# PeterouZh/CIPS-3Dplusplus

Measured on AMD Instinct MI355X. Metric: rendered views/sec at FFHQ 1024^2 (generator forward: 64x64-ray NeRF + StyleGAN2 decoder), higher is better.
Workload: dtype f32 (split-fp16 MFMA products x3, f32 accumulate and storage); 1 GPU; ffhq_r1024_nerf64x64x24_D2_B1_fp32; img_size=64, n_samples=24, N_layers_renderer=2, resolution=1024, parallelism=views x1, views_in_flight=2

## Files before the change

### cips_3dplusplus_amd/csrc/chain.hip

```cpp
#include "mfma_frag.h"

namespace {

#ifdef CIPS3D_CHAIN_STAMPS
__device__ unsigned long long g_chain_stamps[8];
extern "C" int cips3d_debug_read_chain_stamps(unsigned long long* out8) {
  hipDeviceSynchronize();
  hipMemcpyFromSymbol(out8, HIP_SYMBOL(g_chain_stamps), 64);
  unsigned long long z[8] = {0};
  hipMemcpyToSymbol(HIP_SYMBOL(g_chain_stamps), z, 64);
  return 0;
}
#define CSTAMP(i) ts_[i] = __builtin_amdgcn_s_memtime()
#else
#define CSTAMP(i)
#endif

struct ChainArgs {
  const _Float16* x;
  const float* wmp;
  void* out;
  int out_fmt;
  int B, Cin, Cout; int HW;
  int epilogue; const float* noise; int64_t noise_bstride; const float* noise_w; const float* bias;
  const float* rgb_w; float* rgb_part;
  const int* x_exp; int x_exp_const; const float* x_pmax; float x_max_const; const float* lconst; float* out_amax; int* out_exp;
  float* out_pmax;
  cips3d_reduce_job ride;
};



template <int WM, int WGM, int WGN, int BK, int NS, int NP = 2>
__global__ void __launch_bounds__(64 * WGM * WGN) chain_gemm_kernel(ChainArgs a) {
#ifdef CIPS3D_CHAIN_STAMPS
  unsigned long long ts_[6];
  CSTAMP(0);
#endif
  constexpr int NW = WGM * WGN;
  constexpr int BM = 16 * WM * WGM, BN = 64 * WGN;
  constexpr int A_STAGE = BM * BK * NP / 2, B_STAGE = BK * BN * NP / 2, STAGE = A_STAGE + B_STAGE;
  constexpr int A_PIECES = A_STAGE / 256, B_PIECES = B_STAGE / 256, PIECES = A_PIECES + B_PIECES;
  constexpr int PW = PIECES / NW;
  constexpr int KB = BK / 32, KQ = KB * NP;
  static_assert(PIECES % NW == 0 && BK % 32 == 0, "tile shape");
  static_assert(NP != 2 || BN == CIPS3D_PLANES_EXP_BLOCK, "one planes exponent per workgroup pixel block");
  __shared__ __attribute__((aligned(16))) float lds[NS * STAGE];

  const int tid = threadIdx.x;
  const int wave = __builtin_amdgcn_readfirstlane(tid >> 6);
  const int lane = tid & 63;
  const int wm_i = wave / WGN, wn_i = wave % WGN;
  const int q = lane >> 4, col = lane & 15;
  const int b = blockIdx.z;

  if constexpr (NP == 2) {
    if (a.ride.part && (int)blockIdx.y == a.Cout / BM) {
      constexpr int RIDE_K = 12;
      const int64_t wv = ((int64_t)blockIdx.z * gridDim.x + blockIdx.x) * NW + wave;
      const int64_t ride_i = wv * 16 + col;
      const bool ride_on = ride_i < a.ride.n4;
      f32x4 rsl[RIDE_K], rsk = {0.f, 0.f, 0.f, 0.f};
#pragma unroll
      for (int k = 0; k < RIDE_K; ++k)
        rsl[k] = (ride_on && q + 4 * k < a.ride.n_slots)
                     ? *reinterpret_cast<const f32x4*>(a.ride.part + (q + 4 * k) * a.ride.slot_stride + ride_i * 4)
                     : f32x4{0.f, 0.f, 0.f, 0.f};
      if (ride_on && a.ride.skip && q == 0) rsk = *reinterpret_cast<const f32x4*>(a.ride.skip + ride_i * 4);
      f32x4 v = {0.f, 0.f, 0.f, 0.f};
#pragma unroll
      for (int it = 0; it < RIDE_K / 4; ++it)
        if (q + 16 * it < a.ride.n_slots) {
#pragma unroll
          for (int u = 0; u < 4; ++u)
#pragma unroll
            for (int c = 0; c < 4; ++c) v[c] += rsl[4 * it + u][c];
        }
#pragma unroll
      for (int g = 1; g < 4; ++g)
#pragma unroll
        for (int c = 0; c < 4; ++c) {
          const float o = __shfl(v[c], col + 16 * g, 64);
          if (q == 0) v[c] += o;
        }
      if (ride_on && q == 0) {
        const int ch = (int)((ride_i / a.ride.HW4) % 3);
        float bs = 0.f;
        for (int k = 0; k < a.ride.n_bias; ++k) bs += a.ride.bias[k][ch];
#pragma unroll
        for (int c = 0; c < 4; ++c) v[c] += bs;
        if (a.ride.skip) {
#pragma unroll
          for (int c = 0; c < 4; ++c) v[c] += rsk[c];
        }
        *reinterpret_cast<f32x4*>(a.ride.out + ride_i * 4) = v;
      }
      return;
    }
  }
  const int m0 = blockIdx.y * BM, n0 = blockIdx.x * BN;
  const int HW = a.HW, K = a.Cin;
  const int nstage = K / BK;
  float* s_part = lds + (nstage % NS) * STAGE;
  const _Float16* xb = a.x + (int64_t)b * K * HW * NP;
  const float* ab = a.wmp + (int64_t)b * a.Cout * K * NP / 2;

  auto stage_load = [&](int st) {
    float* dstA = lds + (st % NS) * STAGE;
    float* dstB = dstA + A_STAGE;
    const int k0 = st * BK;
#pragma unroll
    for (int j = 0; j < PW; ++j) {
      const int piece = j * NW + wave;
      if (piece < A_PIECES) {
        const int ot_l = piece / KQ, kq_l = piece % KQ;
        const char* ub = reinterpret_cast<const char*>(ab + ((((m0 >> 4) + ot_l) * ((K >> 5) * NP) + (k0 >> 5) * NP + kq_l) * 256));
        unsigned vo = lane * 16;
        asm volatile("" : "+s"(ub), "+v"(vo));
        __builtin_amdgcn_global_load_lds((const __attribute__((address_space(1))) void*)(ub + vo),
                                         (__attribute__((address_space(3))) void*)(dstA + piece * 256), 16, 0, 0);
      } else {
        const int pb = piece - A_PIECES;
        const int row = pb / (BN / 64), chunk = pb % (BN / 64);
        int n = n0 + chunk * 64 + lane;
        if (n > HW - 1) n = HW - 1;
        const char* ub = reinterpret_cast<const char*>(xb + ((int64_t)((k0 >> 3) * NP + row) * HW) * 8);
        unsigned vo = (unsigned)n * 16u;
        asm volatile("" : "+s"(ub), "+v"(vo));
        __builtin_amdgcn_global_load_lds((const __attribute__((address_space(1))) void*)(ub + vo),
                                         (__attribute__((address_space(3))) void*)(dstB + pb * 256), 16, 0, 0);
      }
    }
  };

  const int nl = wn_i * 64 + col;
  int npx[4];
#pragma unroll
  for (int c = 0; c < 4; ++c) npx[c] = n0 + nl + 16 * c;

  float nz[4] = {0.f, 0.f, 0.f, 0.f};
  f32x4 bias4[WM];
  f32x4 wrgb[WM][3];
  float nw = 0.f;
  float kin = NP == 2 ? kSplitInv : 1.f;
  float kout = 1.f, kback = 1.f;
  float lc0 = 0.f, lc1 = 0.f;
  float pin = 0.f;
  const bool track = NP == 2 && a.out_fmt == 1 && a.lconst;
  int e_raw = 0;
  f32x4 lc_raw = {0.f, 0.f, 0.f, 0.f};
  auto issue_ops = [&]() {
    if constexpr (NP == 2) {
      const int nblk = (HW + BN - 1) / BN;
      if (a.x_exp) {
        typedef const __attribute__((address_space(1))) int gi32_t;
        e_raw = __hip_atomic_load(reinterpret_cast<gi32_t*>(reinterpret_cast<uintptr_t>(a.x_exp + b * nblk + blockIdx.x)),
                                  __ATOMIC_RELAXED, __HIP_MEMORY_SCOPE_AGENT);
      }
      if (track) {
        const float* lc = a.lconst + b * 4;
        lc_raw = f32x4{lc[0], lc[1], lc[2], 0.f};
        if (a.x_pmax) {
          const int n_half = (HW + 63) / 64, per = K >> 4;
          const int n_ent = (2 * (int)blockIdx.x + 1 < n_half ? 2 : 1) * per;
          const float* pp = a.x_pmax + ((int64_t)b * n_half + 2 * blockIdx.x) * per;
          if (lane < n_ent) pin = pp[lane];
        }
      }
    }
    if (a.epilogue == 1) {
      if (a.noise && a.noise_w) {
        nw = a.noise_w[0];
        const float* nzp = a.noise + (int64_t)b * a.noise_bstride;
#pragma unroll
        for (int c = 0; c < 4; ++c)
          if (npx[c] < HW) nz[c] = nzp[npx[c]];
      }
#pragma unroll
      for (int i = 0; i < WM; ++i)
        bias4[i] = *reinterpret_cast<const f32x4*>(a.bias + m0 + (wm_i * WM + i) * 16 + 4 * q);
    }
    if (a.rgb_part) {
#pragma unroll
      for (int i = 0; i < WM; ++i)
#pragma unroll
        for (int ch = 0; ch < 3; ++ch)
          wrgb[i][ch] = *reinterpret_cast<const f32x4*>(a.rgb_w + (int64_t)b * 3 * a.Cout + ch * a.Cout + m0 + (wm_i * WM + i) * 16 + 4 * q);
    }
  };
  auto finish_ops = [&]() {
    if constexpr (NP == 2) {
      const int e_in = a.x_exp ? __builtin_amdgcn_readfirstlane(e_raw) : a.x_exp_const;
      kin = cips3d_uniform(kin * cips3d_pow2(e_in));
      if (track) {
        lc0 = lc_raw[0];
        lc1 = fmaxf(lc_raw[1], 1.41421356237309515f * lc_raw[2]);
        if (a.x_pmax) {
          const int n_half = (HW + 63) / 64, per = K >> 4;
          const int n_ent = (2 * (int)blockIdx.x + 1 < n_half ? 2 : 1) * per;
          const float* pp = a.x_pmax + ((int64_t)b * n_half + 2 * blockIdx.x) * per;
          for (int i = lane + 64; i < n_ent; i += 64) pin = fmaxf(pin, pp[i]);
        } else {
          pin = a.x_max_const > 0.f ? a.x_max_const : cips3d_pow2(e_in + 15);
        }
      }
    }
  };
  f32x4 acc[WM][4];
#pragma unroll
  for (int i = 0; i < WM; ++i)
#pragma unroll
    for (int c = 0; c < 4; ++c) acc[i][c] = f32x4{0.f, 0.f, 0.f, 0.f};

  static_assert(NS >= 2 && (NS - 2) * PW <= 63, "counted vmcnt");
  if (NS > 2) issue_ops();
#pragma unroll
  for (int s0 = 0; s0 < NS - 1; ++s0)
    if (s0 < nstage) stage_load(s0);
  if (NS == 2) issue_ops();

#ifdef CIPS3D_CHAIN_STAMPS
  unsigned long long ph_[4] = {0, 0, 0, 0}, tp_ = __builtin_amdgcn_s_memtime();
#define PSTAMP(i) do { const unsigned long long t_ = __builtin_amdgcn_s_memtime(); ph_[i] += t_ - tp_; tp_ = t_; } while (0)
#else
#define PSTAMP(i)
#endif
  for (int st = 0; st < nstage; ++st) {
    int younger = nstage - 1 - st;
    if (younger > NS - 2) younger = NS - 2;
    switch (younger) {
      case 0: __builtin_amdgcn_s_waitcnt(vmcnt_imm(0)); break;
      case 1: __builtin_amdgcn_s_waitcnt(vmcnt_imm(PW)); break;
      case 2: __builtin_amdgcn_s_waitcnt(vmcnt_imm(2 * PW)); break;
      case 3: __builtin_amdgcn_s_waitcnt(vmcnt_imm(3 * PW)); break;
      case 4: __builtin_amdgcn_s_waitcnt(vmcnt_imm(4 * PW)); break;
      default: __builtin_amdgcn_s_waitcnt(vmcnt_imm(5 * PW)); break;
    }
    __builtin_amdgcn_s_barrier();
#ifdef CIPS3D_CHAIN_STAMPS
    if (st == 0) CSTAMP(1);
#endif
    if (st + NS - 1 < nstage) stage_load(st + NS - 1);
    PSTAMP(1);
    const float* sA = lds + (st % NS) * STAGE;
    const float* sB = sA + A_STAGE;
    if constexpr (NP == 2) {
      h8 ah[KB][WM], al[KB][WM], bh[KB][4], bl[KB][4];
#pragma unroll
      for (int kb = 0; kb < KB; ++kb) {
#pragma unroll
        for (int i = 0; i < WM; ++i) {
          ah[kb][i] = *reinterpret_cast<const h8*>(sA + ((wm_i * WM + i) * KQ + 2 * kb) * 256 + lane * 4);
          al[kb][i] = *reinterpret_cast<const h8*>(sA + ((wm_i * WM + i) * KQ + 2 * kb + 1) * 256 + lane * 4);
        }
#pragma unroll
        for (int c = 0; c < 4; ++c) {
          bh[kb][c] = *reinterpret_cast<const h8*>(sB + (((kb * 4 + q) * 2 + 0) * BN + nl + 16 * c) * 4);
          bl[kb][c] = *reinterpret_cast<const h8*>(sB + (((kb * 4 + q) * 2 + 1) * BN + nl + 16 * c) * 4);
        }
      }
      __builtin_amdgcn_sched_barrier(0);
#pragma unroll
      for (int kb = 0; kb < KB; ++kb)
#pragma unroll
        for (int i = 0; i < WM; ++i)
#pragma unroll
          for (int c = 0; c < 4; ++c) {
            acc[i][c] = __builtin_amdgcn_mfma_f32_16x16x32_f16(al[kb][i], bh[kb][c], acc[i][c], 0, 0, 0);
            acc[i][c] = __builtin_amdgcn_mfma_f32_16x16x32_f16(ah[kb][i], bl[kb][c], acc[i][c], 0, 0, 0);
            acc[i][c] = __builtin_amdgcn_mfma_f32_16x16x32_f16(ah[kb][i], bh[kb][c], acc[i][c], 0, 0, 0);
          }
    } else {
      bf8 af[KB][WM], bf[KB][4];
#pragma unroll
      for (int kb = 0; kb < KB; ++kb) {
#pragma unroll
        for (int i = 0; i < WM; ++i)
          af[kb][i] = *reinterpret_cast<const bf8*>(sA + ((wm_i * WM + i) * KQ + kb) * 256 + lane * 4);
#pragma unroll
        for (int c = 0; c < 4; ++c)
          bf[kb][c] = *reinterpret_cast<const bf8*>(sB + ((kb * 4 + q) * BN + nl + 16 * c) * 4);
      }
      __builtin_amdgcn_sched_barrier(0);
#pragma unroll
      for (int kb = 0; kb < KB; ++kb)
#pragma unroll
        for (int i = 0; i < WM; ++i)
#pragma unroll
          for (int c = 0; c < 4; ++c)
            acc[i][c] = __builtin_amdgcn_mfma_f32_16x16x32_bf16(af[kb][i], bf[kb][c], acc[i][c], 0, 0, 0);
    }
    PSTAMP(2);
    asm volatile("s_waitcnt lgkmcnt(0)" ::: "memory");
  }

  CSTAMP(2);
  finish_ops();
  if (track) {
    const float m_in = cips3d_wave_max_uniform(pin);
    const int e = cips3d_split_exp(fmaf(lc1, m_in * 1.000001f, lc0));
    kout = cips3d_uniform(cips3d_pow2(-e));
    kback = cips3d_uniform(cips3d_pow2(e));
    if (blockIdx.y == 0 && tid == 0) a.out_exp[b * ((HW + BN - 1) / BN) + blockIdx.x] = e;
  }
  float prgb[WM][3][4];
#pragma unroll
  for (int i = 0; i < WM; ++i)
#pragma unroll
    for (int ch = 0; ch < 3; ++ch)
#pragma unroll
      for (int c = 0; c < 4; ++c) prgb[i][ch][c] = 0.f;
  const float kact = 1.41421356237309515f * kout;
  const float kpre = a.epilogue == 1 ? kin : kin * kout;
  float mx = 0.f;
#pragma unroll
  for (int i = 0; i < WM; ++i) {
    const int obase = m0 + (wm_i * WM + i) * 16;
#pragma unroll
    for (int c = 0; c < 4; ++c) {
      float v[4];
#pragma unroll
      for (int r = 0; r < 4; ++r) {
        v[r] = acc[i][c][r] * kpre;
        if (a.epilogue == 1) v[r] = lrelu02(fmaf(nw, nz[c], v[r]) + bias4[i][r]) * kact;
      }
      mx = fmaxf(fmaxf(fabsf(v[0]), fabsf(v[1])), fmaxf(fmaxf(fabsf(v[2]), fabsf(v[3])), mx));
      if (a.rgb_part) {
#pragma unroll
        for (int ch = 0; ch < 3; ++ch)
#pragma unroll
          for (int r = 0; r < 4; ++r)
            asm volatile("v_fmac_f32 %0, %1, %2" : "+v"(prgb[i][ch][c]) : "v"(wrgb[i][ch][r]), "v"(v[r]));
      }
      if (npx[c] < HW) {
        if (a.out_fmt == 1) {
          h4 hi, lo;
          split_frag(v[0], v[1], v[2], v[3], hi, lo);
          _Float16* dst = reinterpret_cast<_Float16*>(a.out) +
                          ((((int64_t)b * (a.Cout >> 3) + (obase >> 3) + (q >> 1)) * 2) * HW + npx[c]) * 8 + 4 * (q & 1);
          cips3d_store_wt8(dst, hi);
          cips3d_store_wt8(dst + (int64_t)HW * 8, lo);
        } else if (a.out_fmt == 3) {
          unsigned short* dst = reinterpret_cast<unsigned short*>(a.out) +
                                (((int64_t)b * (a.Cout >> 3) + (obase >> 3) + (q >> 1)) * HW + npx[c]) * 8 + 4 * (q & 1);
          cips3d_store_wt8(dst, pack_bf16(v[0], v[1], v[2], v[3]));
        } else if (a.out_fmt == 2) {
          unsigned short* dst = reinterpret_cast<unsigned short*>(a.out) + ((int64_t)b * a.Cout + obase + 4 * q) * HW + npx[c];
          typedef __bf16 bf16x2_t __attribute__((ext_vector_type(2)));
          typedef float f32x2_t __attribute__((ext_vector_type(2)));
#pragma unroll
          for (int r = 0; r < 4; r += 2) {
            const bf16x2_t p = __builtin_convertvector(f32x2_t{v[r], v[r + 1]}, bf16x2_t);
            const unsigned bits = __builtin_bit_cast(unsigned, p);
            dst[(int64_t)r * HW] = (unsigned short)(bits & 0xffffu);
            dst[(int64_t)(r + 1) * HW] = (unsigned short)(bits >> 16);
          }
        } else {
          float* dst = reinterpret_cast<float*>(a.out) + ((int64_t)b * a.Cout + obase + 4 * q) * HW + npx[c];
#pragma unroll
          for (int r = 0; r < 4; ++r) cips3d_store_wt(dst + (int64_t)r * HW, v[r]);
        }
      }
    }
  }
#ifdef CIPS3D_CHAIN_STAMPS
  CSTAMP(3);
  __builtin_amdgcn_s_waitcnt(vmcnt_imm(0));
  CSTAMP(4);
  if (tid == 0) {
    for (int i = 0; i < 4; ++i) atomicAdd(&g_chain_stamps[i], ts_[i + 1] - ts_[i]);
    atomicAdd(&g_chain_stamps[7], 1ull);
    atomicAdd(&g_chain_stamps[4], ph_[0]);
    atomicAdd(&g_chain_stamps[5], ph_[1]);
    atomicAdd(&g_chain_stamps[6], ph_[2]);
  }
#endif
  if (a.out_pmax && n0 + wn_i * 64 < HW) {
    static_assert(BN == 64 * WGN, "a wave column = one 64-pixel half block");
    const float m = cips3d_wave_max_uniform(mx * kback);
    if (lane < WM)
      a.out_pmax[((int64_t)b * ((HW + 63) / 64) + (n0 >> 6) + wn_i) * (a.Cout >> 4) + (m0 >> 4) + wm_i * WM + lane] = m;
  }
  if (a.out_amax) {
    const float m = cips3d_workgroup_max(mx * kback, s_part, wave, lane, NW);
    if (tid == 0) cips3d_amax_raise_if(a.out_amax + b * CIPS3D_AMAX_FLOATS, m, blockIdx.y * gridDim.x + blockIdx.x);
  }
  if (!a.rgb_part) return;
#pragma unroll
  for (int i = 0; i < WM; ++i)
#pragma unroll
    for (int ch = 0; ch < 3; ++ch)
#pragma unroll
      for (int c = 0; c < 4; ++c) {
        float v = prgb[i][ch][c] * kback;
        v += __shfl_xor(v, 16, 64);
        v += __shfl_xor(v, 32, 64);
        prgb[i][ch][c] = v;
      }
  __syncthreads();
  float* s_red = lds;
  if (q == 0) {
#pragma unroll
    for (int i = 0; i < WM; ++i)
#pragma unroll
      for (int ch = 0; ch < 3; ++ch)
#pragma unroll
        for (int c = 0; c < 4; ++c) s_red[((wm_i * WM + i) * 3 + ch) * BN + nl + 16 * c] = prgb[i][ch][c];
  }
  __syncthreads();
  constexpr int SLOTS = BM / 64;
  static_assert(WGM * WM == 4 * SLOTS, "four tiles per ToRGB slot");
  if (wm_i < SLOTS && q < 3) {
#pragma unroll
    for (int c = 0; c < 4; ++c) {
      if (npx[c] >= HW) continue;
      float v = 0.f;
#pragma unroll
      for (int m = 0; m < 4; ++m) v += s_red[((wm_i * 4 + m) * 3 + q) * BN + nl + 16 * c];
      cips3d_store_wt(a.rgb_part + (((int64_t)blockIdx.y * SLOTS + wm_i) * a.B + b) * 3 * HW + ((int64_t)q * HW + npx[c]), v);
    }
  }
}

__device__ __forceinline__ float amax_of_sample(const float* __restrict__ slots) {
  float m = 0.f;
  for (int s_ = 0; s_ < CIPS3D_AMAX_SLOTS; ++s_) m = fmaxf(m, slots[s_ * CIPS3D_AMAX_STRIDE]);
  return m;
}

__global__ void __launch_bounds__(256) to_planes_kernel(const float* __restrict__ x, _Float16* __restrict__ p, int B, int C,
                                                        int HW, const float* __restrict__ x_amax, int* __restrict__ exp_out,
                                                        float* __restrict__ pmax_out) {
  const int64_t total = (int64_t)B * (C / 8) * HW, per = (int64_t)(C / 8) * HW;
  for (int64_t i = (int64_t)blockIdx.x * blockDim.x + threadIdx.x; i < total; i += (int64_t)gridDim.x * blockDim.x) {
    const int n = (int)(i % HW);
    const int64_t bc = i / HW;
    float k = 1.f;
    if (x_amax) {
      const int b = (int)(i / per);
      const int e_ = cips3d_split_exp(amax_of_sample(x_amax + (int64_t)b * CIPS3D_AMAX_FLOATS));
      k = cips3d_pow2(-e_);
      const int nblk = (HW + CIPS3D_PLANES_EXP_BLOCK - 1) / CIPS3D_PLANES_EXP_BLOCK;
      if (i - b * per < nblk) exp_out[b * nblk + (int)(i - b * per)] = e_;
      if (pmax_out) {
        const int n_pm = ((HW + 63) / 64) * (C >> 4);
        const float am = amax_of_sample(x_amax + (int64_t)b * CIPS3D_AMAX_FLOATS);
        for (int64_t j = i - b * per; j < n_pm; j += per) pmax_out[(int64_t)b * n_pm + j] = am;
      }
    }
    h8 hi, lo;
#pragma unroll
    for (int e = 0; e < 8; ++e) {
      const float v = x[(bc * 8 + e) * HW + n] * k;
      _Float16 h_, l_;
      cips3d_split16(v, h_, l_);
      hi[e] = h_;
      lo[e] = l_;
    }
    *reinterpret_cast<h8*>(p + ((bc * 2) * HW + n) * 8) = hi;
    *reinterpret_cast<h8*>(p + ((bc * 2 + 1) * HW + n) * 8) = lo;
  }
}

__global__ void __launch_bounds__(256) from_planes_kernel(const _Float16* __restrict__ p, float* __restrict__ x, int B, int C,
                                                          int HW, const int* __restrict__ exps) {
  const int64_t total = (int64_t)B * (C / 8) * HW, per = (int64_t)(C / 8) * HW;
  for (int64_t i = (int64_t)blockIdx.x * blockDim.x + threadIdx.x; i < total; i += (int64_t)gridDim.x * blockDim.x) {
    const int n = (int)(i % HW);
    const int64_t bc = i / HW;
    const float k = exps ? cips3d_pow2(exps[(i / per) * ((HW + CIPS3D_PLANES_EXP_BLOCK - 1) / CIPS3D_PLANES_EXP_BLOCK) +
                                            n / CIPS3D_PLANES_EXP_BLOCK]) : 1.f;
    const h8 hi = *reinterpret_cast<const h8*>(p + ((bc * 2) * HW + n) * 8);
    const h8 lo = *reinterpret_cast<const h8*>(p + ((bc * 2 + 1) * HW + n) * 8);
#pragma unroll
    for (int e = 0; e < 8; ++e) x[(bc * 8 + e) * HW + n] = ((float)hi[e] + (float)lo[e]) * k;
  }
}

__global__ void __launch_bounds__(256) to_planes16_kernel(const float* __restrict__ x, unsigned short* __restrict__ p, int B,
                                                          int C, int HW) {
  typedef __bf16 bf16x2_t __attribute__((ext_vector_type(2)));
  typedef float f32x2_t __attribute__((ext_vector_type(2)));
  typedef unsigned u32x4_t __attribute__((ext_vector_type(4)));
  const int64_t total = (int64_t)B * (C / 8) * HW;
  for (int64_t i = (int64_t)blockIdx.x * blockDim.x + threadIdx.x; i < total; i += (int64_t)gridDim.x * blockDim.x) {
    const int n = (int)(i % HW);
    const int64_t bc = i / HW;
    u32x4_t w;
#pragma unroll
    for (int e = 0; e < 8; e += 2) {
      const bf16x2_t pr = __builtin_convertvector(f32x2_t{x[(bc * 8 + e) * HW + n], x[(bc * 8 + e + 1) * HW + n]}, bf16x2_t);
      w[e >> 1] = __builtin_bit_cast(unsigned, pr);
    }
    *reinterpret_cast<u32x4_t*>(p + (bc * HW + n) * 8) = w;
  }
}

__global__ void __launch_bounds__(256) from_planes16_kernel(const unsigned short* __restrict__ p, float* __restrict__ x, int B,
                                                            int C, int HW) {
  typedef unsigned u32x4_t __attribute__((ext_vector_type(4)));
  const int64_t total = (int64_t)B * (C / 8) * HW;
  for (int64_t i = (int64_t)blockIdx.x * blockDim.x + threadIdx.x; i < total; i += (int64_t)gridDim.x * blockDim.x) {
    const int n = (int)(i % HW);
    const int64_t bc = i / HW;
    const u32x4_t w = *reinterpret_cast<const u32x4_t*>(p + (bc * HW + n) * 8);
#pragma unroll
    for (int e = 0; e < 8; e += 2) {
      x[(bc * 8 + e) * HW + n] = __uint_as_float(w[e >> 1] << 16);
      x[(bc * 8 + e + 1) * HW + n] = __uint_as_float(w[e >> 1] & 0xffff0000u);
    }
  }
}

}

extern "C" int cips3d_planes_supported(int Cin, int Cout, int64_t HW) {
  return Cin > 0 && Cout > 0 && Cin % 64 == 0 && Cout % 64 == 0 && HW >= 16 &&
         (int64_t)(Cin > Cout ? Cin : Cout) * HW * 2 + 1024 < ((int64_t)1 << 31);
}

extern "C" int cips3d_planes_torgb_blocks(int Cout) { return Cout > 0 ? Cout / 64 : 0; }

extern "C" int cips3d_to_planes(const float* x, void* planes, int B, int C, int64_t HW, const float* x_amax, int32_t* exp_out,
                                float* pmax_out, void* stream) {
  if (!x || !planes || B < 0 || C <= 0 || HW <= 0 || ((x_amax == nullptr) != (exp_out == nullptr)) || (pmax_out && !x_amax))
    return CIPS3D_E_BADARG;
  if (pmax_out && C % 16 != 0) return CIPS3D_E_UNSUPP;
  if (C % 8 != 0) return CIPS3D_E_UNSUPP;
  if (B == 0) return 0;
  int64_t blocks = ceil_div<int64_t>((int64_t)B * (C / 8) * HW, 256);
  if (blocks > 16384) blocks = 16384;
  hipLaunchKernelGGL(to_planes_kernel, dim3((unsigned)blocks), dim3(256), 0, as_stream(stream), x,
                     reinterpret_cast<_Float16*>(planes), B, C, (int)HW, x_amax, exp_out, pmax_out);
  return cips3d_launch_status();
}

extern "C" int cips3d_from_planes(const void* planes, float* x, int B, int C, int64_t HW, const int32_t* exp, void* stream) {
  if (!x || !planes || B < 0 || C <= 0 || HW <= 0) return CIPS3D_E_BADARG;
  if (C % 8 != 0) return CIPS3D_E_UNSUPP;
  if (B == 0) return 0;
  int64_t blocks = ceil_div<int64_t>((int64_t)B * (C / 8) * HW, 256);
  if (blocks > 16384) blocks = 16384;
  hipLaunchKernelGGL(from_planes_kernel, dim3((unsigned)blocks), dim3(256), 0, as_stream(stream),
                     reinterpret_cast<const _Float16*>(planes), x, B, C, (int)HW, exp);
  return cips3d_launch_status();
}

extern "C" int cips3d_to_planes16(const float* x, void* planes16, int B, int C, int64_t HW, void* stream) {
  if (!x || !planes16 || B < 0 || C <= 0 || HW <= 0) return CIPS3D_E_BADARG;
  if (C % 8 != 0) return CIPS3D_E_UNSUPP;
  if (B == 0) return 0;
  int64_t blocks = ceil_div<int64_t>((int64_t)B * (C / 8) * HW, 256);
  if (blocks > 16384) blocks = 16384;
  hipLaunchKernelGGL(to_planes16_kernel, dim3((unsigned)blocks), dim3(256), 0, as_stream(stream), x,
                     reinterpret_cast<unsigned short*>(planes16), B, C, (int)HW);
  return cips3d_launch_status();
}

extern "C" int cips3d_from_planes16(const void* planes16, float* x, int B, int C, int64_t HW, void* stream) {
  if (!x || !planes16 || B < 0 || C <= 0 || HW <= 0) return CIPS3D_E_BADARG;
  if (C % 8 != 0) return CIPS3D_E_UNSUPP;
  if (B == 0) return 0;
  int64_t blocks = ceil_div<int64_t>((int64_t)B * (C / 8) * HW, 256);
  if (blocks > 16384) blocks = 16384;
  hipLaunchKernelGGL(from_planes16_kernel, dim3((unsigned)blocks), dim3(256), 0, as_stream(stream),
                     reinterpret_cast<const unsigned short*>(planes16), x, B, C, (int)HW);
  return cips3d_launch_status();
}

extern "C" int cips3d_modconv1x1_planes16(const void* x_planes16, const float* wm, void* out, int out_format, int B, int Cin,
                                          int Cout, int64_t HW, int epilogue, const float* noise, int64_t noise_bstride,
                                          const float* noise_w, const float* bias, const float* rgb_w, float* rgb_part,
                                          int* n_row_blocks, const cips3d_range* rg, void* stream) {
  if ((rgb_w == nullptr) != (rgb_part == nullptr)) return CIPS3D_E_BADARG;
  if (n_row_blocks) *n_row_blocks = cips3d_planes_torgb_blocks(Cout);
  if (!x_planes16 || !wm || !out || B < 0 || Cin <= 0 || Cout <= 0 || HW <= 0) return CIPS3D_E_BADARG;
  if ((out_format != 0 && out_format != 2 && out_format != 3) || (epilogue != 0 && epilogue != 1) || (epilogue == 1 && !bias))
    return CIPS3D_E_BADARG;
  if (!cips3d_planes_supported(Cin, Cout, HW)) return CIPS3D_E_UNSUPP;
  if (B == 0) return 0;
  ChainArgs a{reinterpret_cast<const _Float16*>(x_planes16), wm, out, out_format, B, Cin, Cout, (int)HW, epilogue, noise,
              noise_bstride, noise_w, bias, rgb_w, rgb_part, nullptr, 0, nullptr, 0.f, nullptr, rg ? rg->out_amax : nullptr, nullptr,
              nullptr, cips3d_reduce_job{}};
  if (rg && rg->ride) return CIPS3D_E_UNSUPP;
  dim3 grid((unsigned)ceil_div<int64_t>(HW, 128), (unsigned)(Cout / 64), (unsigned)B);
  hipLaunchKernelGGL((chain_gemm_kernel<1, 4, 2, 64, 3, 1>), grid, dim3(512), 0, as_stream(stream), a);
  return cips3d_launch_status();
}

extern "C" int cips3d_modconv1x1_planes(const void* x_planes, const float* wm, void* out, int out_format, int B, int Cin,
                                        int Cout, int64_t HW, int epilogue, const float* noise, int64_t noise_bstride,
                                        const float* noise_w, const float* bias, const float* rgb_w, float* rgb_part,
                                        int* n_row_blocks, const cips3d_range* rg, void* stream) {
  if ((rgb_w == nullptr) != (rgb_part == nullptr)) return CIPS3D_E_BADARG;
  if (n_row_blocks) *n_row_blocks = cips3d_planes_torgb_blocks(Cout);
  if (!x_planes || !wm || !out || B < 0 || Cin <= 0 || Cout <= 0 || HW <= 0) return CIPS3D_E_BADARG;
  if (out_format < 0 || out_format > 2 || (epilogue != 0 && epilogue != 1) || (epilogue == 1 && !bias)) return CIPS3D_E_BADARG;
  if (!cips3d_planes_supported(Cin, Cout, HW)) return CIPS3D_E_UNSUPP;
  if (B == 0) return 0;
  if (rg && out_format == 1 && (!rg->lconst || !rg->out_exp)) return CIPS3D_E_BADARG;
  ChainArgs a{reinterpret_cast<const _Float16*>(x_planes), wm, out, out_format, B, Cin, Cout, (int)HW, epilogue, noise,
              noise_bstride, noise_w, bias, rgb_w, rgb_part, rg ? rg->x_exp : nullptr, rg ? rg->x_exp_const : 0,
              rg ? rg->x_pmax : nullptr, rg ? rg->x_max_const : 0.f, (rg && out_format == 1) ? rg->lconst : nullptr,
              (rg && out_format != 1) ? rg->out_amax : nullptr, rg ? rg->out_exp : nullptr,
              (rg && out_format == 1) ? rg->out_pmax : nullptr, cips3d_reduce_job{}};
  if (rg && out_format == 1 && rg->x_pmax && Cin > 512) return CIPS3D_E_UNSUPP;
  if (rg && rg->ride) {
    const cips3d_reduce_job& j = *rg->ride;
    if (!j.part || !j.out || j.n_slots < 1 || j.n_bias < 0 || j.n_bias > CIPS3D_TORGB_FOLD_MAX || j.n4 <= 0 || j.HW4 <= 0 ||
        j.slot_stride <= 0)
      return CIPS3D_E_BADARG;
    if (j.n_slots > 48 || j.n4 > (int64_t)ceil_div<int64_t>(HW, 128) * B * 8 * 16) return CIPS3D_E_UNSUPP;
    a.ride = j;
  }
  const int64_t tiles64 = (int64_t)B * (Cout / 64) * ceil_div<int64_t>(HW, 128);
  if (rg && rg->half_chip && Cout % 128 == 0 && tiles64 > 192 && tiles64 <= 256) {
    dim3 grid2((unsigned)ceil_div<int64_t>(HW, 128), (unsigned)(Cout / 128) + (a.ride.part ? 1u : 0u), (unsigned)B);
    hipLaunchKernelGGL((chain_gemm_kernel<2, 4, 2, 64, 2>), grid2, dim3(512), 0, as_stream(stream), a);
    return cips3d_launch_status();
  }
  dim3 grid((unsigned)ceil_div<int64_t>(HW, 128), (unsigned)(Cout / 64) + (a.ride.part ? 1u : 0u), (unsigned)B);
  hipLaunchKernelGGL((chain_gemm_kernel<1, 4, 2, 64, 2>), grid, dim3(512), 0, as_stream(stream), a);
  return cips3d_launch_status();
}
```

Measured before the change: 3435 views/s.

## Software-pipeline LDS fragment reads with MFMA and precompute DMA source addresses

Restructures the chain GEMM main loop so the split-fp16 path reads the two k-block fragment sets in a ping-pong fashion with inline ds_read_b128 and counted lgkmcnt waits. MFMAs for one k-block overlap the LDS reads of the next, and the last block's MFMAs carry into the following stage. Global-to-LDS load addresses are computed once and advanced by constant strides instead of being recomputed per stage. The loop is also split into a steady-state part with a fixed vmcnt wait and a drain tail. This adds register pressure for two fragment sets, and the hand-written waitcnt bookkeeping is fragile.

```diff
diff --git a/cips_3dplusplus_amd/csrc/chain.hip b/cips_3dplusplus_amd/csrc/chain.hip
--- a/cips_3dplusplus_amd/csrc/chain.hip
+++ b/cips_3dplusplus_amd/csrc/chain.hip
@@ -105,32 +105,40 @@
   const _Float16* xb = a.x + (int64_t)b * K * HW * NP;
   const float* ab = a.wmp + (int64_t)b * a.Cout * K * NP / 2;
 
-  auto stage_load = [&](int st) {
-    float* dstA = lds + (st % NS) * STAGE;
-    float* dstB = dstA + A_STAGE;
-    const int k0 = st * BK;
+  constexpr int AJ = A_PIECES / NW;
+  static_assert(A_PIECES % NW == 0, "a wave's piece j is an A piece for j < AJ, a B piece otherwise, whatever the wave");
+  const char* src[PW];
+  unsigned voff[PW];
+#pragma unroll
+  for (int j = 0; j < PW; ++j) {
+    const int piece = j * NW + wave;
+    if (j < AJ) {
+      const int ot_l = piece / KQ, kq_l = piece % KQ;
+      src[j] = reinterpret_cast<const char*>(ab + ((int64_t)((m0 >> 4) + ot_l) * ((K >> 5) * NP) + kq_l) * 256);
+      voff[j] = lane * 16;
+    } else {
+      const int pb = piece - A_PIECES;
+      const int row = pb / (BN / 64), chunk = pb % (BN / 64);
+      int n = n0 + chunk * 64 + lane;
+      if (n > HW - 1) n = HW - 1;
+      src[j] = reinterpret_cast<const char*>(xb + (int64_t)row * HW * 8);
+      voff[j] = (unsigned)n * 16u;
+    }
+  }
+  const int64_t a_step = (int64_t)KQ * 1024, b_step = (int64_t)(BK / 8) * NP * HW * 16;
+  int ld_slot = 0;
+  auto stage_load = [&]() {
+    float* dst = lds + ld_slot + wave * 256;
 #pragma unroll
     for (int j = 0; j < PW; ++j) {
-      const int piece = j * NW + wave;
-      if (piece < A_PIECES) {
-        const int ot_l = piece / KQ, kq_l = piece % KQ;
-        const char* ub = reinterpret_cast<const char*>(ab + ((((m0 >> 4) + ot_l) * ((K >> 5) * NP) + (k0 >> 5) * NP + kq_l) * 256));
-        unsigned vo = lane * 16;
-        asm volatile("" : "+s"(ub), "+v"(vo));
-        __builtin_amdgcn_global_load_lds((const __attribute__((address_space(1))) void*)(ub + vo),
-                                         (__attribute__((address_space(3))) void*)(dstA + piece * 256), 16, 0, 0);
-      } else {
-        const int pb = piece - A_PIECES;
-        const int row = pb / (BN / 64), chunk = pb % (BN / 64);
-        int n = n0 + chunk * 64 + lane;
-        if (n > HW - 1) n = HW - 1;
-        const char* ub = reinterpret_cast<const char*>(xb + ((int64_t)((k0 >> 3) * NP + row) * HW) * 8);
-        unsigned vo = (unsigned)n * 16u;
-        asm volatile("" : "+s"(ub), "+v"(vo));
-        __builtin_amdgcn_global_load_lds((const __attribute__((address_space(1))) void*)(ub + vo),
-                                         (__attribute__((address_space(3))) void*)(dstB + pb * 256), 16, 0, 0);
-      }
-    }
+      const char* ub = src[j];
+      unsigned vo = voff[j];
+      asm volatile("" : "+s"(ub), "+v"(vo));
+      __builtin_amdgcn_global_load_lds((const __attribute__((address_space(1))) void*)(ub + vo),
+                                       (__attribute__((address_space(3))) void*)(dst + j * NW * 256), 16, 0, 0);
+      src[j] = ub + (j < AJ ? a_step : b_step);
+    }
+    ld_slot = ld_slot + STAGE == NS * STAGE ? 0 : ld_slot + STAGE;
   };
 
   const int nl = wn_i * 64 + col;
@@ -216,7 +224,7 @@
   if (NS > 2) issue_ops();
 #pragma unroll
   for (int s0 = 0; s0 < NS - 1; ++s0)
-    if (s0 < nstage) stage_load(s0);
+    if (s0 < nstage) stage_load();
   if (NS == 2) issue_ops();
 
 #ifdef CIPS3D_CHAIN_STAMPS
@@ -225,10 +233,119 @@
 #else
 #define PSTAMP(i)
 #endif
-  for (int st = 0; st < nstage; ++st) {
-    int younger = nstage - 1 - st;
-    if (younger > NS - 2) younger = NS - 2;
-    switch (younger) {
+  struct Frags {
+    h8 ah[WM], al[WM], bh[4], bl[4];
+  };
+  Frags fp, fq;
+  static_assert(NP != 2 || (KB == 2 && (WM == 1 || WM == 2)), "two fragment sets = the two k-blocks of a stage");
+  constexpr int FRAG_READS = 2 * WM + 8;
+  const unsigned ldsA = (unsigned)(uintptr_t)(__attribute__((address_space(3))) void*)lds + wm_i * WM * KQ * 1024 + lane * 16;
+  const unsigned ldsB = (unsigned)(uintptr_t)(__attribute__((address_space(3))) void*)lds + A_STAGE * 4 + (q * 2 * BN + nl) * 16;
+#define CIPS3D_DS_READ16(dst, addr, off) asm volatile("ds_read_b128 %0, %1 offset:%2" : "=v"(dst) : "v"(addr), "i"(off) : "memory")
+  auto read_frags = [&](Frags& f, unsigned aA, unsigned aB, auto kbc) {
+    constexpr int kb = decltype(kbc)::value;
+#pragma unroll
+    for (int i = 0; i < WM; ++i) {
+      CIPS3D_DS_READ16(f.ah[i], aA, (i * KQ + 2 * kb) * 1024);
+      CIPS3D_DS_READ16(f.al[i], aA, (i * KQ + 2 * kb + 1) * 1024);
+    }
+#pragma unroll
+    for (int c = 0; c < 4; ++c) {
+      CIPS3D_DS_READ16(f.bh[c], aB, (kb * 8 + 0) * BN * 16 + c * 256);
+      CIPS3D_DS_READ16(f.bl[c], aB, (kb * 8 + 1) * BN * 16 + c * 256);
+    }
+  };
+#undef CIPS3D_DS_READ16
+  auto wait_frags = [&](Frags& f, auto newer) {
+    constexpr int n = decltype(newer)::value;
+    static_assert(n <= 15, "lgkmcnt is a 4-bit counter");
+    if constexpr (WM == 2)
+      asm volatile("s_waitcnt lgkmcnt(%12)"
+                   : "+v"(f.ah[0]), "+v"(f.al[0]), "+v"(f.ah[1]), "+v"(f.al[1]), "+v"(f.bh[0]), "+v"(f.bl[0]), "+v"(f.bh[1]),
+                     "+v"(f.bl[1]), "+v"(f.bh[2]), "+v"(f.bl[2]), "+v"(f.bh[3]), "+v"(f.bl[3])
+                   : "n"(n)
+                   : "memory");
+    else
+      asm volatile("s_waitcnt lgkmcnt(%10)"
+                   : "+v"(f.ah[0]), "+v"(f.al[0]), "+v"(f.bh[0]), "+v"(f.bl[0]), "+v"(f.bh[1]), "+v"(f.bl[1]), "+v"(f.bh[2]),
+                     "+v"(f.bl[2]), "+v"(f.bh[3]), "+v"(f.bl[3])
+                   : "n"(n)
+                   : "memory");
+  };
+  auto mfma_frags = [&](const Frags& f) {
+#pragma unroll
+    for (int i = 0; i < WM; ++i)
+#pragma unroll
+      for (int c = 0; c < 4; ++c) acc[i][c] = __builtin_amdgcn_mfma_f32_16x16x32_f16(f.al[i], f.bh[c], acc[i][c], 0, 0, 0);
+#pragma unroll
+    for (int i = 0; i < WM; ++i)
+#pragma unroll
+      for (int c = 0; c < 4; ++c) acc[i][c] = __builtin_amdgcn_mfma_f32_16x16x32_f16(f.ah[i], f.bl[c], acc[i][c], 0, 0, 0);
+#pragma unroll
+    for (int i = 0; i < WM; ++i)
+#pragma unroll
+      for (int c = 0; c < 4; ++c) acc[i][c] = __builtin_amdgcn_mfma_f32_16x16x32_f16(f.ah[i], f.bh[c], acc[i][c], 0, 0, 0);
+  };
+  int rd_slot = 0;
+  auto stage_body = [&](int st, auto dma) {
+    const int slot = rd_slot;
+    rd_slot = rd_slot + STAGE == NS * STAGE ? 0 : rd_slot + STAGE;
+    if constexpr (NP == 2) {
+      const unsigned aA = ldsA + slot * 4, aB = ldsB + slot * 4;
+      read_frags(fp, aA, aB, std::integral_constant<int, 0>{});
+      __builtin_amdgcn_sched_barrier(0);
+      if constexpr (decltype(dma)::value) stage_load();
+      __builtin_amdgcn_sched_barrier(0);
+      PSTAMP(1);
+      if (st > 0) mfma_frags(fq);
+      __builtin_amdgcn_sched_barrier(0);
+      read_frags(fq, aA, aB, std::integral_constant<int, 1>{});
+      wait_frags(fp, std::integral_constant<int, FRAG_READS>{});
+      __builtin_amdgcn_sched_barrier(0);
+      mfma_frags(fp);
+      __builtin_amdgcn_sched_barrier(0);
+      PSTAMP(2);
+      wait_frags(fq, std::integral_constant<int, 0>{});
+      __builtin_amdgcn_sched_barrier(0);
+    } else {
+      const float* sA = lds + slot;
+      const float* sB = sA + A_STAGE;
+      if constexpr (decltype(dma)::value) stage_load();
+      PSTAMP(1);
+      bf8 af[KB][WM], bf[KB][4];
+#pragma unroll
+      for (int kb = 0; kb < KB; ++kb) {
+#pragma unroll
+        for (int i = 0; i < WM; ++i)
+          af[kb][i] = *reinterpret_cast<const bf8*>(sA + ((wm_i * WM + i) * KQ + kb) * 256 + lane * 4);
+#pragma unroll
+        for (int c = 0; c < 4; ++c)
+          bf[kb][c] = *reinterpret_cast<const bf8*>(sB + ((kb * 4 + q) * BN + nl + 16 * c) * 4);
+      }
+      __builtin_amdgcn_sched_barrier(0);
+#pragma unroll
+      for (int kb = 0; kb < KB; ++kb)
+#pragma unroll
+        for (int i = 0; i < WM; ++i)
+#pragma unroll
+          for (int c = 0; c < 4; ++c)
+            acc[i][c] = __builtin_amdgcn_mfma_f32_16x16x32_bf16(af[kb][i], bf[kb][c], acc[i][c], 0, 0, 0);
+      PSTAMP(2);
+      asm volatile("s_waitcnt lgkmcnt(0)" ::: "memory");
+    }
+  };
+  int st = 0;
+  for (; st < nstage - (NS - 1); ++st) {
+    __builtin_amdgcn_s_waitcnt(vmcnt_imm((NS - 2) * PW));
+    __builtin_amdgcn_s_barrier();
+#ifdef CIPS3D_CHAIN_STAMPS
+    if (st == 0) CSTAMP(1);
+#endif
+    PSTAMP(0);
+    stage_body(st, std::true_type{});
+  }
+  for (; st < nstage; ++st) {
+    switch (NS == 2 ? 0 : nstage - 1 - st) {
       case 0: __builtin_amdgcn_s_waitcnt(vmcnt_imm(0)); break;
       case 1: __builtin_amdgcn_s_waitcnt(vmcnt_imm(PW)); break;
       case 2: __builtin_amdgcn_s_waitcnt(vmcnt_imm(2 * PW)); break;
@@ -240,59 +357,10 @@
 #ifdef CIPS3D_CHAIN_STAMPS
     if (st == 0) CSTAMP(1);
 #endif
-    if (st + NS - 1 < nstage) stage_load(st + NS - 1);
-    PSTAMP(1);
-    const float* sA = lds + (st % NS) * STAGE;
-    const float* sB = sA + A_STAGE;
-    if constexpr (NP == 2) {
-      h8 ah[KB][WM], al[KB][WM], bh[KB][4], bl[KB][4];
-#pragma unroll
-      for (int kb = 0; kb < KB; ++kb) {
-#pragma unroll
-        for (int i = 0; i < WM; ++i) {
-          ah[kb][i] = *reinterpret_cast<const h8*>(sA + ((wm_i * WM + i) * KQ + 2 * kb) * 256 + lane * 4);
-          al[kb][i] = *reinterpret_cast<const h8*>(sA + ((wm_i * WM + i) * KQ + 2 * kb + 1) * 256 + lane * 4);
-        }
-#pragma unroll
-        for (int c = 0; c < 4; ++c) {
-          bh[kb][c] = *reinterpret_cast<const h8*>(sB + (((kb * 4 + q) * 2 + 0) * BN + nl + 16 * c) * 4);
-          bl[kb][c] = *reinterpret_cast<const h8*>(sB + (((kb * 4 + q) * 2 + 1) * BN + nl + 16 * c) * 4);
-        }
-      }
-      __builtin_amdgcn_sched_barrier(0);
-#pragma unroll
-      for (int kb = 0; kb < KB; ++kb)
-#pragma unroll
-        for (int i = 0; i < WM; ++i)
-#pragma unroll
-          for (int c = 0; c < 4; ++c) {
-            acc[i][c] = __builtin_amdgcn_mfma_f32_16x16x32_f16(al[kb][i], bh[kb][c], acc[i][c], 0, 0, 0);
-            acc[i][c] = __builtin_amdgcn_mfma_f32_16x16x32_f16(ah[kb][i], bl[kb][c], acc[i][c], 0, 0, 0);
-            acc[i][c] = __builtin_amdgcn_mfma_f32_16x16x32_f16(ah[kb][i], bh[kb][c], acc[i][c], 0, 0, 0);
-          }
-    } else {
-      bf8 af[KB][WM], bf[KB][4];
-#pragma unroll
-      for (int kb = 0; kb < KB; ++kb) {
-#pragma unroll
-        for (int i = 0; i < WM; ++i)
-          af[kb][i] = *reinterpret_cast<const bf8*>(sA + ((wm_i * WM + i) * KQ + kb) * 256 + lane * 4);
-#pragma unroll
-        for (int c = 0; c < 4; ++c)
-          bf[kb][c] = *reinterpret_cast<const bf8*>(sB + ((kb * 4 + q) * BN + nl + 16 * c) * 4);
-      }
-      __builtin_amdgcn_sched_barrier(0);
-#pragma unroll
-      for (int kb = 0; kb < KB; ++kb)
-#pragma unroll
-        for (int i = 0; i < WM; ++i)
-#pragma unroll
-          for (int c = 0; c < 4; ++c)
-            acc[i][c] = __builtin_amdgcn_mfma_f32_16x16x32_bf16(af[kb][i], bf[kb][c], acc[i][c], 0, 0, 0);
-    }
-    PSTAMP(2);
-    asm volatile("s_waitcnt lgkmcnt(0)" ::: "memory");
-  }
+    PSTAMP(0);
+    stage_body(st, std::false_type{});
+  }
+  if constexpr (NP == 2) mfma_frags(fq);
 
   CSTAMP(2);
   finish_ops();
```

After: 3479 views/s (median of 6 runs). 1.01x the previous value.
